# tomdbar/naqs-for-quantum-chemistry

Hardware: AMD Instinct MI355X
Metric: unique samples/sec through E_loc + log-psi eval (N2, 20 qubits) (higher is better)
Workload: dtype f32 network (f16x2-split MFMA, f32-equivalent) / f64 E_loc; 1 GPU; N2 STO-3G (20 qubits, K=2239 Pauli terms, Kxy=378), 10000 unique samples per GPU, 1xMI355X per rank; pipeline=2 independent batches in flight on 2 HIP streams (one handle pair each), batches=4 distinct key sets per rank, rotated every step, input=unique sampled bit-strings (keys) resident in HBM; random-init network, ranks=single process, no process group

## Files before the change

### include/naqs_hip.h

```cpp
#ifndef NAQS_HIP_H
#define NAQS_HIP_H

#include <stdint.h>

#ifdef __cplusplus
extern "C" {
#endif

#define NAQS_ABI_VERSION 9

typedef struct naqs_ham naqs_ham_t;

enum naqs_status {
    NAQS_OK = 0,
    NAQS_ERR_INVALID = -1,
    NAQS_ERR_HIP = -2,
    NAQS_ERR_NOMEM = -3,
    NAQS_ERR_UNSUPPORTED = -4,
    NAQS_ERR_NO_DEVICE = -5
};

enum naqs_psi_kind {
    NAQS_PSI_F32 = 0,
    NAQS_PSI_F64 = 1,
// ... 35 lines not shown

int naqs_hmatvec(naqs_ham_t *h, int64_t M, const uint64_t *keys_dev, const double *v_dev, int64_t row_begin,
                 int64_t n_rows, double *out_dev, void *stream);

int naqs_ham_connected(naqs_ham_t *h, int64_t M, const uint64_t *keys_dev, int64_t row_begin, int64_t n_rows,
                       int64_t capacity, uint64_t *out_keys_dev, int64_t *count_dev, void *stream);


int naqs_popcount_parity(const void *arr_dev, int elem_bytes, int64_t n, int8_t *out_dev, void *stream);

int naqs_get_hij(naqs_ham_t *h, int64_t M, const uint64_t *keys_dev, double *hij_dev, void *stream);

int naqs_hij_from_parity(int64_t M, int64_t Kxy, int64_t Kyz, int64_t K, const int8_t *parity_dev,
                         const int32_t *group_ptr_dev, const int32_t *term_yz_dev, const void *term_coeff_dev,
                         int coeff_bytes, void *hij_dev, void *stream);

int naqs_csr_mv(int64_t rows, const double *data_dev, const int32_t *indices_dev,
                const int32_t *indptr_dev, const double *v_dev, double *out_dev, void *stream);


int naqs_prof_enable(naqs_ham_t *h, int max_records);
int naqs_prof_read(naqs_ham_t *h, double *total_ms, int64_t *launches);
int naqs_ham_last_kernel(const naqs_ham_t *h, char *buf, int buf_len);
int naqs_prof_stride(naqs_ham_t *h, int stride);


typedef struct naqs_net naqs_net_t;

#define NAQS_NET_MAX_PAIRS 16
#define NAQS_NET_MAX_PHASE_LAYERS 8

typedef struct naqs_net_config {
    int32_t n_qubits;
    int32_t n_alpha, n_beta;
    int32_t masking;
    int32_t use_amp_spin_sym;
    int32_t amp_hidden;
    int32_t n_phase_hidden;
    int32_t phase_hidden[NAQS_NET_MAX_PHASE_LAYERS];
    int32_t qubit2model[2 * NAQS_NET_MAX_PAIRS];
    int32_t aggregate_phase;
    int32_t use_phase_spin_sym;
} naqs_net_config_t;

int naqs_net_create(const naqs_net_config_t *cfg, int device, naqs_net_t **out);
int naqs_net_create_amp_layers(const naqs_net_config_t *cfg, int32_t n_amp_hidden, int device, naqs_net_t **out);
// ... 126 lines not shown
```

### naqs-for-quantum-chemistry_amd/csrc/naqs_hip.hip

```cpp

#include <hip/hip_runtime.h>

#include <algorithm>
#include <cmath>
#include <cstdint>
#include <cstdio>
#include <cstdlib>
#include <cstring>
#include <new>
#include <numeric>
#include <type_traits>
#include <vector>

#include "naqs_common.hpp"
#include "naqs_reduce.hpp"
#include "naqs_src_hash.h"
#include "naqs_hash.hpp"
#include "naqs_poll.hpp"

#include <mutex>

namespace naqs {
thread_local hipError_t g_last_hip = hipSuccess;
thread_local char g_last_msg[200] = {0};
std::atomic<int64_t> g_launches{0};
}

namespace {

using naqs::WAVE;
using naqs::DeviceGuard;
using naqs::env_int;

constexpr int BLOCK = 256;
#ifndef NAQS_LIGHT_BATCH
#define NAQS_LIGHT_BATCH 2
#endif
constexpr int LIGHT_BATCH = NAQS_LIGHT_BATCH;
constexpr int LIGHT_BATCH_BLOOM = 4;
constexpr int queue_cap(bool bloom) { return 64 * ((bloom ? LIGHT_BATCH_BLOOM : LIGHT_BATCH) + 1); }
constexpr int LDS_BUDGET = 78 * 1024;
// ... 34 lines not shown
}

template <typename KT>
struct ElocParams {
    const KT *xy_g;
    const int32_t *row_ptr;
    const KT *yz_t;
    const double *c_t;
    int32_t Kxy, K;
    int32_t has_diag;
    int32_t light_begin;
    KT alpha_mask, beta_mask;
    int32_t n_alpha, n_beta;
    const KT *keys;
    const double2 *psi;
    const Slot<KT> *tab;
    int32_t bits;
    uint32_t tag;
    const uint32_t *bloom;
    int64_t row_begin, n_rows;
    int32_t rows_per_block;
    int32_t matvec;
    double2 *eloc;
};

using naqs::wave_sum;

__device__ __forceinline__ uint32_t to_sgpr(uint32_t v) { return (uint32_t)__builtin_amdgcn_readfirstlane((int)v); }
__device__ __forceinline__ uint64_t to_sgpr(uint64_t v) {
    const uint32_t hi = (uint32_t)__builtin_amdgcn_readfirstlane((int)(uint32_t)(v >> 32));
    const uint32_t lo = (uint32_t)__builtin_amdgcn_readfirstlane((int)(uint32_t)v);
    return ((uint64_t)hi << 32) | (uint64_t)lo;
}

__device__ __forceinline__ double2 cdiv(double2 a, double2 b) {
    double2 q;
    if (fabs(b.x) >= fabs(b.y)) {
        const double rat = b.y / b.x, scl = 1.0 / (b.x + b.y * rat);
        q.x = (a.x + a.y * rat) * scl;
        q.y = (a.y - a.x * rat) * scl;
    } else {
        const double rat = b.x / b.y, scl = 1.0 / (b.y + b.x * rat);
        q.x = (a.x * rat + a.y) * scl;
        q.y = (a.y * rat - a.x) * scl;
    }
    return q;
// ... 155 lines not shown
            while (qn >= WAVE) {
                qn -= WAVE;
                drain(qn, true);
                __builtin_amdgcn_wave_barrier();
            }
        }
        drain(0, lane < qn);
        __builtin_amdgcn_wave_barrier();

        sr = wave_sum(sr);
        si = wave_sum(si);
        if (lane == 0) {
            if (p.matvec) {
                p.eloc[r] = make_double2(sr, si);
            } else {
                const double2 q = cdiv(make_double2(sr, si), psi_i);
                p.eloc[r] = make_double2(q.x, -q.y);
            }
        }
    }

}

constexpr int PASS_BATCH = 3;
constexpr int PQ_CAP = 64 * (PASS_BATCH + 1), HQ_CAP = 128;
constexpr size_t queue_bytes_v2(int nwaves) { return (size_t)nwaves * (HQ_CAP * sizeof(int2) + PQ_CAP * sizeof(int32_t)) + 16; }

template <typename KT, int STAGE, int NT, bool BLOOM>
__global__ __launch_bounds__(NT) void eloc_kernel2(const ElocParams<KT> p) {
    constexpr int NWAVES = NT / WAVE;
    extern __shared__ __attribute__((aligned(16))) unsigned char smem[];
    double *s_c = reinterpret_cast<double *>(smem);
    int2 *s_hq = reinterpret_cast<int2 *>(s_c + (STAGE >= 2 ? p.K : 0));
    int32_t *s_pq = reinterpret_cast<int32_t *>(s_hq + NWAVES * HQ_CAP);
    int32_t *s_rp = s_pq + NWAVES * PQ_CAP + 4;
    KT *s_xy = reinterpret_cast<KT *>(s_rp + (STAGE >= 1 ? (p.Kxy + 2) & ~1 : 0));
    KT *s_yz = s_xy + (STAGE >= 1 ? p.Kxy : 0);
    uint32_t *s_bloom = reinterpret_cast<uint32_t *>(
        smem + ((reinterpret_cast<unsigned char *>(s_yz + (STAGE >= 2 ? p.K : 0)) - smem + 15) & ~15ull));

    const int tid = threadIdx.x, lane = tid & (WAVE - 1), wave = tid >> 6;

    if (BLOOM) {
        const uint4 *src = reinterpret_cast<const uint4 *>(p.bloom);
        uint4 *dst = reinterpret_cast<uint4 *>(s_bloom);
#pragma unroll 4
        for (int e = tid; e < BLOOM_WORDS / 4; e += NT) dst[e] = src[e];
    }
    if (STAGE >= 1) {
        const int n_max = STAGE >= 2 ? (p.K > p.Kxy + 1 ? p.K : p.Kxy + 1) : p.Kxy + 1;
#pragma unroll 4
        for (int t = tid; t < n_max; t += NT) {
            const bool gx = t < p.Kxy, gr = t <= p.Kxy, gt = STAGE >= 2 && t < p.K;
            const KT vx = gx ? p.xy_g[t] : (KT)0;
            const int32_t vr = gr ? p.row_ptr[t] : 0;
            KT vy = (KT)0;
            double vc = 0.0;
            if (STAGE >= 2) { vy = gt ? p.yz_t[t] : (KT)0; vc = gt ? p.c_t[t] : 0.0; }
            if (gx) s_xy[t] = vx;
            if (gr) s_rp[t] = vr;
            if (STAGE >= 2 && gt) { s_yz[t] = vy; s_c[t] = vc; }
        }
    }
    __syncthreads();

    const KT *xy = STAGE >= 1 ? s_xy : p.xy_g;
    const int32_t *rp = STAGE >= 1 ? s_rp : p.row_ptr;
    const KT *yz = STAGE >= 2 ? s_yz : p.yz_t;
    const double *cf = STAGE >= 2 ? s_c : p.c_t;
    int2 *hq = s_hq + wave * HQ_CAP;
    int32_t *pq = s_pq + wave * PQ_CAP;

    const int64_t blk_begin = (int64_t)blockIdx.x * p.rows_per_block;
    const int blk_rows = (int)min((int64_t)p.rows_per_block, p.n_rows - blk_begin);
    const bool filter = p.n_alpha >= 0;
    const Slot<KT> *__restrict__ tab = p.tab;
    const double2 *__restrict__ psi = p.psi;

    const int wave_u = __builtin_amdgcn_readfirstlane(wave);
    if (wave_u < blk_rows % NWAVES) __builtin_amdgcn_s_setprio(1);
    for (int rl = wave; rl < blk_rows; rl += NWAVES) {
        const int64_t r = blk_begin + rl;
        const int64_t i = p.row_begin + r;
        const KT key = to_sgpr(p.keys[i]);
        const double2 psi_i = psi[i];
        double sr = 0.0, si = 0.0;

        if (p.has_diag) {
            const double h = sign_sum_strided<KT>(key, yz, cf, rp[0], rp[1], lane);
            sr = h * psi_i.x;
            si = h * psi_i.y;
        }

        int qn = 0, pn = 0;
        auto drain = [&](int first, bool active) {
            if (active) {
                const int2 e = hq[first + lane];
                const double2 pj = psi[e.y];
                const int t0 = e.x & 0xFFFFFF;
                const double h = sign_sum<KT>(key, yz, cf, t0, t0 + (int)((uint32_t)e.x >> 24));
                sr += h * pj.x;
                si += h * pj.y;
            }
        };
        auto push_hits = [&](int g, int idx) {
            const unsigned long long m = __ballot(idx >= 0);
            if (m) {
                if (idx >= 0) {
                    const int pos = qn + __builtin_amdgcn_mbcnt_hi((uint32_t)(m >> 32), __builtin_amdgcn_mbcnt_lo((uint32_t)m, 0));
                    const int t0 = rp[g];
                    hq[pos] = make_int2(t0 | ((rp[g + 1] - t0) << 24), idx);
                }
                qn += __popcll(m);
                __builtin_amdgcn_wave_barrier();
                if (qn >= WAVE) {
                    qn -= WAVE;
                    drain(qn, true);
                    __builtin_amdgcn_wave_barrier();
                }
            }
        };
        auto probe_pass = [&](int first, bool active) {
            int idx = -1, g = 0;
            if (active) {
                g = pq[first + lane];
                const KT j = key ^ xy[g];
                if (!BLOOM || naqs::bloom_test<KT>(s_bloom, j)) idx = hash_find<KT>(tab, p.bits, p.tag, j);
            }
            push_hits(g, idx);
        };
        auto filter_pass = [&](int g, bool in_range) {
            bool ok = false;
            if (in_range) {
                const KT j = key ^ xy[g];
                ok = !filter || (popc((KT)(j & p.alpha_mask)) == p.n_alpha && popc((KT)(j & p.beta_mask)) == p.n_beta);
            }
            const unsigned long long m = __ballot(ok);
            if (ok) pq[pn + __builtin_amdgcn_mbcnt_hi((uint32_t)(m >> 32), __builtin_amdgcn_mbcnt_lo((uint32_t)m, 0))] = g;
            pn += __popcll(m);
        };
        int g0 = p.has_diag;
        for (; g0 + PASS_BATCH * WAVE <= p.Kxy; g0 += PASS_BATCH * WAVE) {
#pragma unroll
            for (int u = 0; u < PASS_BATCH; ++u) filter_pass(g0 + u * WAVE + lane, true);
            __builtin_amdgcn_wave_barrier();
            while (pn >= WAVE) {
                pn -= WAVE;
                probe_pass(pn, true);
            }
        }
        for (; g0 < p.Kxy; g0 += WAVE) {
            filter_pass(g0 + lane, g0 + lane < p.Kxy);
            __builtin_amdgcn_wave_barrier();
            if (pn >= WAVE) {
                pn -= WAVE;
                probe_pass(pn, true);
            }
        }
// ... 207 lines not shown
        const uint32_t n = min(*s_fill, (uint32_t)p.wg_stage);
        if (tid == 0) s_base = n ? atomicAdd(p.count, (unsigned long long)n) : 0ull;
        __syncthreads();
        const unsigned long long base = s_base;
        for (uint32_t i = tid; i < n; i += NT)
            if (base + i < cap) p.out[base + i] = (uint64_t)s_keys[i];
    }
}

}

struct naqs_ham {
    int device = 0;
    char last_kernel[96] = {0};
    int n_qubits = 0, n_alpha = -1, n_beta = -1;
    int key_bits = 32;
    int64_t K = 0, Kxy = 0;
    int32_t has_diag = 0, diag_terms = 0, n_heavy = 0;
    int32_t chunk_terms = 8;
    uint64_t alpha_mask = 0, beta_mask = 0;
    void *d_xy = nullptr, *d_yz = nullptr;
    int32_t *d_rp = nullptr, *d_col = nullptr;
    double *d_c = nullptr;
    int64_t Kxy2 = 0;
    void *d_xy2 = nullptr;
    int32_t *d_rp2 = nullptr;
    int64_t cap_M = 0;
    void *d_keys = nullptr;
    double2 *d_psi = nullptr;
    void *d_tab = nullptr;
    int64_t tab_slots = 0;
    uint32_t epoch = 0;
    uint32_t *d_bloom = nullptr;
    unsigned long long *d_seen = nullptr;
    int64_t seen_slots = 0;
    int64_t *d_conn_count = nullptr;
    int64_t *h_conn = nullptr, *d_conn_alias = nullptr;
    int64_t conn_seq = 0;
    int cu_count = 256;
    naqs::EventRing prof;
};

namespace {

int table_bits(int64_t M, size_t slot_bytes) {
    static const int64_t fmin = std::max(2, env_int("NAQS_TABLE_FACTOR", 4));
    static const int64_t fmax = std::max((int)fmin, env_int("NAQS_TABLE_MAX_FACTOR", 16));
    static const int64_t grow_bytes = (int64_t)std::max(0, env_int("NAQS_TABLE_GROW_KB", 1024)) * 1024;
    int bits = 10;
// ... 26 lines not shown
template <typename KT>
int upload_tables(naqs_ham *h, const std::vector<uint64_t> &xy_g, const std::vector<int32_t> &rp,
                  const std::vector<int32_t> &col, const std::vector<uint64_t> &yz_t,
                  const std::vector<double> &c_t) {
    std::vector<KT> xy_n(xy_g.begin(), xy_g.end()), yz_n(yz_t.begin(), yz_t.end());
    HIP_TRY(hipMalloc(&h->d_xy, std::max<size_t>(1, xy_n.size()) * sizeof(KT)));
    HIP_TRY(hipMalloc(&h->d_yz, std::max<size_t>(1, yz_n.size()) * sizeof(KT)));
    HIP_TRY(hipMalloc((void **)&h->d_rp, rp.size() * sizeof(int32_t)));
    HIP_TRY(hipMalloc((void **)&h->d_col, std::max<size_t>(1, col.size()) * sizeof(int32_t)));
    HIP_TRY(hipMemcpy(h->d_col, col.data(), col.size() * sizeof(int32_t), hipMemcpyHostToDevice));
    HIP_TRY(hipMalloc((void **)&h->d_c, std::max<size_t>(1, c_t.size()) * sizeof(double)));
    HIP_TRY(hipMemcpy(h->d_xy, xy_n.data(), xy_n.size() * sizeof(KT), hipMemcpyHostToDevice));
    HIP_TRY(hipMemcpy(h->d_yz, yz_n.data(), yz_n.size() * sizeof(KT), hipMemcpyHostToDevice));
    HIP_TRY(hipMemcpy(h->d_rp, rp.data(), rp.size() * sizeof(int32_t), hipMemcpyHostToDevice));
    HIP_TRY(hipMemcpy(h->d_c, c_t.data(), c_t.size() * sizeof(double), hipMemcpyHostToDevice));
    {
        const double oa = (double)((h->n_qubits + 1) / 2), ob = (double)(h->n_qubits / 2);
        double log2_states = (double)h->n_qubits;
        if (h->n_alpha >= 0 && h->n_beta >= 0)
            log2_states = (std::lgamma(oa + 1.0) - std::lgamma(h->n_alpha + 1.0) - std::lgamma(oa - h->n_alpha + 1.0) +
                           std::lgamma(ob + 1.0) - std::lgamma(h->n_beta + 1.0) - std::lgamma(ob - h->n_beta + 1.0)) / std::log(2.0);
        h->chunk_terms = std::min(255, std::max(1, env_int("NAQS_CHUNK_TERMS", log2_states > 20.0 ? 64 : HEAVY_TERMS)));
    }
    std::vector<KT> xy2;
    std::vector<int32_t> rp2;
    for (size_t g = 0; g + 1 < rp.size(); ++g) {
        const int32_t step = (int32_t)g < h->has_diag ? rp[g + 1] - rp[g] : h->chunk_terms;
        for (int32_t t = rp[g]; t < rp[g + 1]; t += std::max(step, 1)) { xy2.push_back(xy_n[g]); rp2.push_back(t); }
    }
    rp2.push_back(rp.back());
    h->Kxy2 = (int64_t)xy2.size();
    HIP_TRY(hipMalloc(&h->d_xy2, std::max<size_t>(1, xy2.size()) * sizeof(KT)));
    HIP_TRY(hipMalloc((void **)&h->d_rp2, rp2.size() * sizeof(int32_t)));
    HIP_TRY(hipMemcpy(h->d_xy2, xy2.data(), xy2.size() * sizeof(KT), hipMemcpyHostToDevice));
    HIP_TRY(hipMemcpy(h->d_rp2, rp2.data(), rp2.size() * sizeof(int32_t), hipMemcpyHostToDevice));
    HIP_TRY(hipDeviceSynchronize());
    return NAQS_OK;
}

int eloc_begin_impl(naqs_ham *h, int64_t M, hipStream_t s, naqs::ElocFeed *feed) {
    int st = ensure_scratch(h, M);
    if (st != NAQS_OK) return st;
    const size_t slot = h->key_bits == 32 ? sizeof(Slot<uint32_t>) : sizeof(Slot<uint64_t>);
    if (++h->epoch > 255u) {
        HIP_TRY(hipMemsetAsync(h->d_tab, 0, (size_t)h->tab_slots * slot, s));
        h->epoch = 1;
    }
    const int bloom_env = env_int("NAQS_BLOOM", -1);
    const bool use_bloom = bloom_env >= 0 ? bloom_env != 0 : (M >= 20000);
    feed->bloom = nullptr;
    if (use_bloom) {
        if (!h->d_bloom) HIP_TRY(hipMalloc((void **)&h->d_bloom, BLOOM_WORDS * sizeof(uint32_t)));
        HIP_TRY(hipMemsetAsync(h->d_bloom, 0, BLOOM_WORDS * sizeof(uint32_t), s));
        feed->bloom = h->d_bloom;
    }
    feed->tab = h->d_tab;
    feed->keys_narrow = h->d_keys;
// ... 17 lines not shown
template <typename KT>
int launch_main(naqs_ham *h, int64_t M, const naqs::ElocFeed &f, int64_t row_begin, int64_t n_rows, double *eloc_dev,
                const double *w_dev, double *out4_dev, hipStream_t s, bool matvec = false) {
    const int bits = f.bits;
    const uint32_t tag = f.tag;
    auto *tab = reinterpret_cast<Slot<KT> *>(f.tab);

    ElocParams<KT> p;
    p.xy_g = reinterpret_cast<const KT *>(h->d_xy);
    p.row_ptr = h->d_rp;
    p.yz_t = reinterpret_cast<const KT *>(h->d_yz);
    p.c_t = h->d_c;
    p.Kxy = (int32_t)h->Kxy; p.K = (int32_t)h->K;
    p.has_diag = h->has_diag;
    p.light_begin = h->has_diag + h->n_heavy;
    p.alpha_mask = (KT)h->alpha_mask; p.beta_mask = (KT)h->beta_mask;
    p.n_alpha = h->n_alpha; p.n_beta = h->n_beta;
    p.keys = reinterpret_cast<const KT *>(h->d_keys);
    p.psi = h->d_psi;
    p.tab = tab; p.bits = bits; p.tag = tag;
    p.row_begin = row_begin; p.n_rows = n_rows;
    p.eloc = reinterpret_cast<double2 *>(eloc_dev);
    p.matvec = matvec ? 1 : 0;

    const int ver = env_int("NAQS_ELOC_V", 2);
    const bool v2 = ver != 1 && h->K < (1 << 24);
    int nt = env_int("NAQS_BLOCK", 0);
    if (nt != 256 && nt != 512 && nt != 1024) nt = n_rows >= 1024 ? 1024 : 512;
    const int nwaves = nt / WAVE;
    int rpb = env_int("NAQS_ROWS_PER_BLOCK", 0);
    if (rpb <= 0) {
        const int64_t target_blocks = (int64_t)h->cu_count * (2048 / nt);
        rpb = (int)std::max<int64_t>(nwaves, (n_rows + target_blocks - 1) / target_blocks);
    }
    p.rows_per_block = rpb;

    const bool bloom = f.bloom != nullptr && nt == 1024;
    p.bloom = bloom ? f.bloom : nullptr;
    const size_t b_bytes = bloom ? (size_t)BLOOM_WORDS * sizeof(uint32_t) + 16 : 0;
    const size_t budget = bloom ? (size_t)LDS_BUDGET_BLOOM : (size_t)LDS_BUDGET;
    if (bloom) {
        const int64_t target_blocks = (int64_t)h->cu_count;
        if (env_int("NAQS_ROWS_PER_BLOCK", 0) <= 0)
            rpb = (int)std::max<int64_t>(nwaves, (n_rows + target_blocks - 1) / target_blocks);
        p.rows_per_block = rpb;
    }
    const int grid2 = (int)((n_rows + rpb - 1) / rpb);
    const int64_t Kxy_k = v2 ? h->Kxy2 : h->Kxy;
    if (v2) { p.xy_g = reinterpret_cast<const KT *>(h->d_xy2); p.row_ptr = h->d_rp2; p.Kxy = (int32_t)h->Kxy2; }
    const size_t q_bytes = v2 ? queue_bytes_v2(nwaves) : (size_t)nwaves * queue_cap(bloom) * sizeof(int2) + 16;
    const size_t g_bytes = (size_t)((Kxy_k + 2) & ~1ll) * sizeof(int32_t) + (size_t)Kxy_k * sizeof(KT);
    const size_t t_bytes = (size_t)h->K * (sizeof(double) + sizeof(KT));
    const int force = env_int("NAQS_STAGE", -1);
    int stage = (q_bytes + g_bytes + t_bytes + b_bytes <= budget) ? 2 : (q_bytes + g_bytes + b_bytes <= budget ? 1 : 0);
    if (force >= 0 && force < stage) stage = force;
    const size_t lds = q_bytes + (stage >= 1 ? g_bytes : 0) + (stage >= 2 ? t_bytes : 0) + b_bytes;

    const bool prof = h->prof.armed();
    if (prof) { int st = h->prof.begin(s); if (st != NAQS_OK) return st; }
#define NAQS_LAUNCH_K(KERNEL, ST, NTHREADS, BL)                                                                     \
    do {                                                                                                            \
        if (lds > 64 * 1024)                                               \
            (void)hipFuncSetAttribute(reinterpret_cast<const void *>(&KERNEL<KT, ST, NTHREADS, BL>),                \
                                      hipFuncAttributeMaxDynamicSharedMemorySize, (int)budget);                      \
        NAQS_KLAUNCH((KERNEL<KT, ST, NTHREADS, BL>), dim3(grid2), dim3(NTHREADS), lds, s, p);                 \
    } while (0)
#define NAQS_LAUNCH(ST, NTHREADS, BL)                                                                               \
    do {                                                                                                            \
        if (v2) NAQS_LAUNCH_K(eloc_kernel2, ST, NTHREADS, BL);                                                 \
        else NAQS_LAUNCH_K(eloc_kernel, ST, NTHREADS, BL);                                                          \
    } while (0)
#define NAQS_LAUNCH_NT(ST)                                          \
    do {                                                            \
        if (bloom) NAQS_LAUNCH(ST, 1024, true);                     \
        else if (nt == 1024) NAQS_LAUNCH(ST, 1024, false);          \
// ... 204 lines not shown
            c_d[(size_t)pos] = c_t[(size_t)t];
        }
    }
    rp_d[(size_t)Kxy] = pos;

    DeviceGuard guard;
    st = guard.init(device);
    if (st == NAQS_OK) {
        hipDeviceProp_t prop;
        if (hipGetDeviceProperties(&prop, device) == hipSuccess) h->cu_count = prop.multiProcessorCount;
        st = h->key_bits == 32 ? upload_tables<uint32_t>(h, xy_d, rp_d, col, yz_d, c_d)
                               : upload_tables<uint64_t>(h, xy_d, rp_d, col, yz_d, c_d);
    }
    if (st != NAQS_OK) { naqs_ham_destroy(h); return st; }
    *out = h;
    return NAQS_OK;
}

NAQS_API int naqs_ham_destroy(naqs_ham_t *h) {
    if (!h) return NAQS_OK;
    DeviceGuard guard;
    (void)guard.init(h->device);
    (void)h->prof.enable(0);
    void *ptrs[] = {h->d_xy, h->d_yz, h->d_rp, h->d_col, h->d_c, h->d_xy2, h->d_rp2, h->d_keys, h->d_psi, h->d_tab, h->d_bloom, h->d_seen};
    for (void *p : ptrs) if (p) (void)hipFree(p);
    if (h->d_conn_count) (void)hipFree(h->d_conn_count);
    if (h->h_conn) (void)hipHostFree(h->h_conn);
    delete h;
    return NAQS_OK;
}

NAQS_API int naqs_ham_info(const naqs_ham_t *h, int64_t info[8]) {
    if (!h || !info) return NAQS_ERR_INVALID;
    info[0] = h->K; info[1] = h->Kxy; info[2] = h->n_qubits; info[3] = h->n_alpha; info[4] = h->n_beta;
    info[5] = h->key_bits; info[6] = h->diag_terms; info[7] = h->device;
    return NAQS_OK;
}

NAQS_API int naqs_ham_reserve(naqs_ham_t *h, int64_t M) {
    if (!h || M < 0) return NAQS_ERR_INVALID;
    if (M >= (1ll << 31)) return NAQS_ERR_UNSUPPORTED;
    DeviceGuard guard;
    int st = guard.init(h->device);
    if (st != NAQS_OK) return st;
    return ensure_scratch(h, M);
}

static int eloc_common(naqs_ham_t *h, int64_t M, const uint64_t *keys_dev, const void *psi_dev, int psi_kind,
                       int64_t row_begin, int64_t n_rows, double *eloc_dev, const double *w_dev, double *out4_dev,
                       void *stream, bool matvec = false, int64_t S = 0, int64_t S_pad = 0) {
    if (!h || M < 0 || row_begin < 0 || n_rows < 0 || row_begin + n_rows > M) return NAQS_ERR_INVALID;
    if (psi_kind < NAQS_PSI_F32 || psi_kind > NAQS_LOGPSI_F64) return NAQS_ERR_INVALID;
    if (M > (int64_t)IDX_MASK) return NAQS_ERR_UNSUPPORTED;
    if ((w_dev == nullptr) != (out4_dev == nullptr)) return NAQS_ERR_INVALID;
    hipStream_t s = reinterpret_cast<hipStream_t>(stream);
    DeviceGuard guard;
    int st = guard.init(h->device);
    if (st != NAQS_OK) return st;
// ... 328 lines not shown
```

### naqs-for-quantum-chemistry_amd/naqs_amd/_lib.py

```python
import ctypes
import os

_HERE = os.path.dirname(os.path.abspath(__file__))
_LIB_DIR = os.path.join(os.path.dirname(_HERE), "lib")

NAQS_OK = 0
ABI_VERSION = 9
PSI_F32, PSI_F64, LOGPSI_F32, LOGPSI_F64 = 0, 1, 2, 3

c_i64, c_u64p, c_f64p, c_vp = ctypes.c_int64, ctypes.POINTER(ctypes.c_uint64), ctypes.POINTER(ctypes.c_double), ctypes.c_void_p

SIGNATURES = {
    "naqs_abi_version": (ctypes.c_int, []),
    "naqs_source_hash": (ctypes.c_char_p, []),
    "naqs_strerror": (ctypes.c_char_p, [ctypes.c_int]),
    "naqs_last_hip_error": (ctypes.c_int, []),
    "naqs_last_hip_error_string": (ctypes.c_char_p, []),
    "naqs_device_count": (ctypes.c_int, []),
    "naqs_device_check": (ctypes.c_int, [ctypes.c_int]),
    "naqs_net_check": (ctypes.c_int, [c_vp]),
    "naqs_terms_group": (ctypes.c_int, [c_i64, c_vp, c_vp, c_vp, ctypes.POINTER(c_i64), c_vp, c_vp, c_vp, c_vp, c_vp]),
    "naqs_ham_create": (ctypes.c_int, [ctypes.c_int, ctypes.c_int, ctypes.c_int, c_i64, c_vp, c_vp, c_vp,
                                       ctypes.c_int, ctypes.POINTER(c_vp)]),
    "naqs_ham_destroy": (ctypes.c_int, [c_vp]),
    "naqs_ham_info": (ctypes.c_int, [c_vp, ctypes.POINTER(c_i64 * 8)]),
    "naqs_ham_reserve": (ctypes.c_int, [c_vp, c_i64]),
    "naqs_eloc": (ctypes.c_int, [c_vp, c_i64, c_vp, c_vp, ctypes.c_int, c_i64, c_i64, c_vp, c_vp]),
    "naqs_eloc_reduced": (ctypes.c_int, [c_vp, c_i64, c_vp, c_vp, ctypes.c_int, c_i64, c_i64, c_vp, c_vp, c_vp, c_vp]),
    "naqs_eloc_reduce": (ctypes.c_int, [c_vp, c_i64, c_vp, c_vp, c_vp, c_vp]),
    "naqs_hmatvec": (ctypes.c_int, [c_vp, c_i64, c_vp, c_vp, c_i64, c_i64, c_vp, c_vp]),
    "naqs_ham_connected": (ctypes.c_int, [c_vp, c_i64, c_vp, c_i64, c_i64, c_i64, c_vp, c_vp, c_vp]),
    "naqs_exact_eloc": (ctypes.c_int, [c_vp, c_vp, c_i64, c_vp, c_vp, c_i64, c_i64, c_i64, c_vp, c_vp, c_vp, ctypes.POINTER(c_i64), c_vp]),
    "naqs_popcount_parity": (ctypes.c_int, [c_vp, ctypes.c_int, c_i64, c_vp, c_vp]),
    "naqs_get_hij": (ctypes.c_int, [c_vp, c_i64, c_vp, c_vp, c_vp]),
    "naqs_hij_from_parity": (ctypes.c_int, [c_i64, c_i64, c_i64, c_i64, c_vp, c_vp, c_vp, c_vp, ctypes.c_int, c_vp, c_vp]),
    "naqs_csr_mv": (ctypes.c_int, [c_i64, c_vp, c_vp, c_vp, c_vp, c_vp, c_vp]),
    "naqs_ham_last_kernel": (ctypes.c_int, [c_vp, ctypes.c_char_p, ctypes.c_int]),
    "naqs_net_last_kernel": (ctypes.c_int, [c_vp, ctypes.c_char_p, ctypes.c_int]),
    "naqs_prof_enable": (ctypes.c_int, [c_vp, ctypes.c_int]),
    "naqs_prof_read": (ctypes.c_int, [c_vp, ctypes.POINTER(ctypes.c_double), ctypes.POINTER(c_i64)]),
    "naqs_prof_stride": (ctypes.c_int, [c_vp, ctypes.c_int]),
    "naqs_net_prof_stride": (ctypes.c_int, [c_vp, ctypes.c_int]),
    "naqs_net_create": (ctypes.c_int, [c_vp, ctypes.c_int, ctypes.POINTER(c_vp)]),
    "naqs_net_create_amp_layers": (ctypes.c_int, [c_vp, ctypes.c_int32, ctypes.c_int, ctypes.POINTER(c_vp)]),
    "naqs_net_create_combined": (ctypes.c_int, [c_vp, ctypes.c_int, ctypes.POINTER(c_vp)]),
    "naqs_net_create_agg_layers": (ctypes.c_int, [c_vp, ctypes.c_int32, ctypes.c_int, ctypes.POINTER(c_vp)]),
    "naqs_net_destroy": (ctypes.c_int, [c_vp]),
    "naqs_net_param_count": (ctypes.c_int, [c_vp, ctypes.POINTER(c_i64)]),
    "naqs_net_set_weights": (ctypes.c_int, [c_vp, c_vp, c_i64, c_vp]),
    "naqs_net_logpsi": (ctypes.c_int, [c_vp, c_i64, c_vp, c_vp, c_vp]),
    "naqs_logpsi_eloc": (ctypes.c_int, [c_vp, c_vp, c_i64, c_vp, c_vp, c_vp, c_vp, c_vp, c_vp]),
    "naqs_net_prof_enable": (ctypes.c_int, [c_vp, ctypes.c_int]),
    "naqs_net_prof_read": (ctypes.c_int, [c_vp, ctypes.POINTER(ctypes.c_double), ctypes.POINTER(c_i64)]),
    "naqs_net_sample": (ctypes.c_int, [c_vp, c_i64, ctypes.c_uint64, c_i64, c_vp, c_vp, c_vp, c_vp, c_vp]),
    "naqs_net_sample_weighted": (ctypes.c_int, [c_vp, c_i64, ctypes.c_uint64, c_i64, c_vp, c_vp, c_vp, c_vp, c_vp, c_vp]),
    "naqs_net_amp_param_count": (ctypes.c_int, [c_vp, ctypes.POINTER(c_i64)]),
    "naqs_net_set_amp_weights": (ctypes.c_int, [c_vp, c_vp, c_i64, c_vp]),
    "naqs_net_logamp": (ctypes.c_int, [c_vp, c_i64, c_vp, c_vp, c_vp]),
    "naqs_net_amp_backward": (ctypes.c_int, [c_vp, c_i64, c_vp, c_vp, c_vp, c_vp]),
    "naqs_net_train_forward": (ctypes.c_int, [c_vp, c_i64, c_vp, c_vp, c_vp]),
# ... 111 lines not shown
```

### naqs-for-quantum-chemistry_amd/naqs_amd/hamiltonian.py

```python
import ctypes

import numpy as np
import torch

from . import _lib
from .packing import PackedHamiltonian, pack_qubit_hamiltonian

_KIND = {("psi", torch.float32): _lib.PSI_F32, ("psi", torch.float64): _lib.PSI_F64,
         ("log_psi", torch.float32): _lib.LOGPSI_F32, ("log_psi", torch.float64): _lib.LOGPSI_F64}


def _stream_ptr(device):
    return ctypes.c_void_p(torch.cuda.current_stream(device).cuda_stream)


def keys_to_device(keys, device):
    if isinstance(keys, np.ndarray):
        keys = torch.from_numpy(np.ascontiguousarray(keys).astype(np.uint64).view(np.int64))
    keys = keys.reshape(-1)
    if keys.dtype != torch.int64:
        keys = keys.to(torch.int64)
    return keys.to(device).contiguous()


# ... 190 lines not shown

    def dense_hij(self, keys):
        M = keys.shape[0]
        out = torch.empty((M, self.Kxy), dtype=torch.float64, device=self.device)
        st = self._lib.naqs_get_hij(self._h, M, keys.contiguous().data_ptr(), out.data_ptr(),
                                    _stream_ptr(self.device))
        _lib.check(st, "naqs_get_hij")
        return out

    def prof_enable(self, max_records, stride=1):
        _lib.check(self._lib.naqs_prof_enable(self._h, int(max_records)), "naqs_prof_enable")
        _lib.check(self._lib.naqs_prof_stride(self._h, int(stride)), "naqs_prof_stride")

    def prof_read(self):
        ms, n = ctypes.c_double(0), ctypes.c_int64(0)
        _lib.check(self._lib.naqs_prof_read(self._h, ctypes.byref(ms), ctypes.byref(n)), "naqs_prof_read")
        return ms.value, n.value

    def last_kernel(self):
        buf = ctypes.create_string_buffer(128)
        _lib.check(self._lib.naqs_ham_last_kernel(self._h, buf, 128), "naqs_ham_last_kernel")
        return buf.value.decode()


def popcount_parity_device(arr):
    if arr.dtype not in (torch.int16, torch.int32, torch.int64):
        raise TypeError(f"Unsupported array dtype for popcount_parity(...): {arr.dtype}.")
    lib = _lib.load_library()
    a = arr.contiguous()
    out = torch.empty(a.shape if a.dim() > 1 else (a.numel(), 1), dtype=torch.int8, device=a.device)
    st = lib.naqs_popcount_parity(a.data_ptr(), a.element_size(), a.numel(), out.data_ptr(), _stream_ptr(a.device))
    _lib.check(st, "naqs_popcount_parity")
    return out


def csr_mv_device(data, indices, indptr, v):
    lib = _lib.load_library()
    rows = indptr.numel() - 1
    out = torch.empty((rows, 2), dtype=torch.float64, device=v.device)
    st = lib.naqs_csr_mv(rows, data.contiguous().data_ptr(), indices.contiguous().data_ptr(),
                         indptr.contiguous().data_ptr(), v.contiguous().data_ptr(), out.data_ptr(),
                         _stream_ptr(v.device))
    _lib.check(st, "naqs_csr_mv")
    return out


# ... 49 lines not shown
```

Baseline: 352.2 million unique samples/s.

## Precompute closed-form sign tables for Pauli groups in local energy kernel

Classifies each off-diagonal Pauli group (4-flip groups whose YZ masks share a common reference, and 2-flip groups with at most one extra spectator bit) and precomputes per-group lookup tables of summed signed coefficients. At evaluation time these groups replace a per-term parity loop with one or a few table loads plus a reference parity. It also repacks the remaining terms into a compact per-chunk layout, uses a single-exit hash probe, and simplifies the electron-count filter to a total popcount. The cost is extra table memory read from global memory, added per-lane branching, and host-side classification at setup.

```diff
diff --git a/include/naqs_hip.h b/include/naqs_hip.h
--- a/include/naqs_hip.h
+++ b/include/naqs_hip.h
@@ -81,6 +81,9 @@
 int naqs_prof_enable(naqs_ham_t *h, int max_records);
 int naqs_prof_read(naqs_ham_t *h, double *total_ms, int64_t *launches);
 int naqs_ham_last_kernel(const naqs_ham_t *h, char *buf, int buf_len);
+int naqs_ham_closed_counts(const naqs_ham_t *h, int64_t out[4]);
+int naqs_closed_group(int n_qubits, uint64_t xy, int64_t n_terms, const uint64_t *yz, const double *coeff,
+                      int32_t *class_out, uint64_t *ref_out, double *table_out);
 int naqs_prof_stride(naqs_ham_t *h, int stride);
 
 
diff --git a/naqs-for-quantum-chemistry_amd/csrc/naqs_closed.hpp b/naqs-for-quantum-chemistry_amd/csrc/naqs_closed.hpp
--- /dev/null
+++ b/naqs-for-quantum-chemistry_amd/csrc/naqs_closed.hpp
@@ -0,0 +1,86 @@
+#pragma once
+#include <algorithm>
+#include <cstdint>
+#include <vector>
+
+namespace naqs {
+namespace closed {
+
+constexpr int SEG_BITS = 6;
+constexpr int SEG_SIZE = 1 << SEG_BITS;
+constexpr int MAX_UNITS = 1 << 12;
+constexpr int MAX_CLASSIFY_TERMS = 4096;
+enum { CLASS_L = 0, CLASS_D = 1, CLASS_S = 2 };
+
+struct Group {
+    int cls = CLASS_L;
+    uint64_t R = 0;
+    int pos[4] = {0, 0, 0, 0};
+};
+
+inline int popc64(uint64_t v) { return __builtin_popcountll(v); }
+inline int n_segments(int n_qubits) { return (n_qubits + SEG_BITS - 1) / SEG_BITS; }
+inline size_t d_table_doubles() { return 16; }
+inline size_t s_table_doubles(int nseg) { return (size_t)4 * (size_t)nseg * SEG_SIZE; }
+
+inline uint64_t deposit(const Group &g, int pattern, int nflip) {
+    uint64_t m = 0;
+    for (int i = 0; i < nflip; ++i)
+        if ((pattern >> i) & 1) m |= 1ull << g.pos[i];
+    return m;
+}
+
+inline Group classify(uint64_t xy, const uint64_t *yz, int n) {
+    Group g;
+    const int nflip = popc64(xy);
+    if ((nflip != 2 && nflip != 4) || n <= 0 || n > MAX_CLASSIFY_TERMS) return g;
+    int best = 1 << 30, ref = 0;
+    for (int r = 0; r < n; ++r) {
+        int worst = 0;
+        for (int t = 0; t < n; ++t) worst = std::max(worst, popc64((yz[t] ^ yz[r]) & ~xy));
+        if (worst < best) { best = worst; ref = r; }
+    }
+    if (!((nflip == 4 && best == 0) || (nflip == 2 && best <= 1))) return g;
+    g.cls = nflip == 4 ? CLASS_D : CLASS_S;
+    g.R = yz[ref];
+    for (int q = 0, k = 0; q < 64; ++q)
+        if ((xy >> q) & 1) g.pos[k++] = q;
+    return g;
+}
+
+inline uint32_t d_word(const Group &g) {
+    return (uint32_t)g.pos[0] | (uint32_t)g.pos[1] << 6 | (uint32_t)g.pos[2] << 12 | (uint32_t)g.pos[3] << 18;
+}
+inline uint32_t s_word(const Group &g, int unit) {
+    return (uint32_t)g.pos[0] | (uint32_t)g.pos[1] << 6 | (uint32_t)unit << 12;
+}
+
+inline void build_d(const Group &g, const uint64_t *yz, const double *c, int n, double *T) {
+    for (int p = 0; p < 16; ++p) {
+        const uint64_t dep = deposit(g, p, 4);
+        double acc = 0.0;
+        for (int t = 0; t < n; ++t) acc += (popc64(dep & (yz[t] ^ g.R)) & 1) ? -c[t] : c[t];
+        T[p] = acc;
+    }
+}
+
+inline void build_s(const Group &g, uint64_t xy, const uint64_t *yz, const double *c, int n, int nseg, double *B) {
+    for (int p = 0; p < 4; ++p) {
+        const uint64_t dep = deposit(g, p, 2);
+        for (int s = 0; s < nseg; ++s)
+            for (int v = 0; v < SEG_SIZE; ++v) {
+                double acc = 0.0;
+                for (int t = 0; t < n; ++t) {
+                    const uint64_t d = yz[t] ^ g.R, sp = d & ~xy;
+                    const int r = sp ? __builtin_ctzll(sp) : 0;
+                    if (r / SEG_BITS != s) continue;
+                    const int par = popc64(dep & d) + (sp ? (v >> (r - s * SEG_BITS)) & 1 : 0);
+                    acc += (par & 1) ? -c[t] : c[t];
+                }
+                B[((size_t)s * 4 + p) * SEG_SIZE + v] = acc;
+            }
+    }
+}
+
+}
+}
diff --git a/naqs-for-quantum-chemistry_amd/csrc/naqs_hip.hip b/naqs-for-quantum-chemistry_amd/csrc/naqs_hip.hip
--- a/naqs-for-quantum-chemistry_amd/csrc/naqs_hip.hip
+++ b/naqs-for-quantum-chemistry_amd/csrc/naqs_hip.hip
@@ -17,6 +17,7 @@
 #include "naqs_src_hash.h"
 #include "naqs_hash.hpp"
 #include "naqs_poll.hpp"
+#include "naqs_closed.hpp"
 
 #include <mutex>
 
@@ -97,6 +98,8 @@
     int32_t rows_per_block;
     int32_t matvec;
     double2 *eloc;
+    const double *tbl;
+    int32_t n_ref, nseg;
 };
 
 using naqs::wave_sum;
@@ -298,6 +301,25 @@
 
 }
 
+__device__ __forceinline__ uint32_t slot_val(unsigned long long kv) { return (uint32_t)kv; }
+__device__ __forceinline__ uint32_t slot_val(const naqs::Slot64Val &s) { return s.val; }
+__device__ __forceinline__ bool slot_has(unsigned long long kv, uint32_t key) { return (uint32_t)(kv >> 32) == key; }
+__device__ __forceinline__ bool slot_has(const naqs::Slot64Val &s, uint64_t key) { return s.key == key; }
+template <typename KT>
+__device__ __forceinline__ int hash_find_one_exit(const Slot<KT> *__restrict__ tab, int bits, uint32_t tag, KT key) {
+    const uint32_t mask = (1u << bits) - 1u;
+    uint32_t h = hash_key(key, bits);
+    auto s = probe_load(tab, h);
+    for (;;) {
+        const uint32_t val = slot_val(s);
+        const bool current = (val & ~IDX_MASK) == tag, hit = current && slot_has(s, key);
+        if (!current || hit) return hit ? (int)(val & IDX_MASK) : -1;
+        h = (h + 1) & mask;
+        s = probe_load(tab, h);
+    }
+}
+
+constexpr int S_BATCH = 4;
 constexpr int PASS_BATCH = 3;
 constexpr int PQ_CAP = 64 * (PASS_BATCH + 1), HQ_CAP = 128;
 constexpr size_t queue_bytes_v2(int nwaves) { return (size_t)nwaves * (HQ_CAP * sizeof(int2) + PQ_CAP * sizeof(int32_t)) + 16; }
@@ -311,7 +333,7 @@
     int32_t *s_pq = reinterpret_cast<int32_t *>(s_hq + NWAVES * HQ_CAP);
     int32_t *s_rp = s_pq + NWAVES * PQ_CAP + 4;
     KT *s_xy = reinterpret_cast<KT *>(s_rp + (STAGE >= 1 ? (p.Kxy + 2) & ~1 : 0));
-    KT *s_yz = s_xy + (STAGE >= 1 ? p.Kxy : 0);
+    KT *s_yz = s_xy + (STAGE >= 1 ? p.Kxy + p.n_ref : 0);
     uint32_t *s_bloom = reinterpret_cast<uint32_t *>(
         smem + ((reinterpret_cast<unsigned char *>(s_yz + (STAGE >= 2 ? p.K : 0)) - smem + 15) & ~15ull));
 
@@ -324,10 +346,11 @@
         for (int e = tid; e < BLOOM_WORDS / 4; e += NT) dst[e] = src[e];
     }
     if (STAGE >= 1) {
-        const int n_max = STAGE >= 2 ? (p.K > p.Kxy + 1 ? p.K : p.Kxy + 1) : p.Kxy + 1;
+        const int n_xy = p.Kxy + p.n_ref;
+        const int n_max = STAGE >= 2 ? (p.K > n_xy + 1 ? p.K : n_xy + 1) : n_xy + 1;
 #pragma unroll 4
         for (int t = tid; t < n_max; t += NT) {
-            const bool gx = t < p.Kxy, gr = t <= p.Kxy, gt = STAGE >= 2 && t < p.K;
+            const bool gx = t < n_xy, gr = t <= p.Kxy, gt = STAGE >= 2 && t < p.K;
             const KT vx = gx ? p.xy_g[t] : (KT)0;
             const int32_t vr = gr ? p.row_ptr[t] : 0;
             KT vy = (KT)0;
@@ -344,12 +367,14 @@
     const int32_t *rp = STAGE >= 1 ? s_rp : p.row_ptr;
     const KT *yz = STAGE >= 2 ? s_yz : p.yz_t;
     const double *cf = STAGE >= 2 ? s_c : p.c_t;
+    const double *__restrict__ tbl = p.tbl;
     int2 *hq = s_hq + wave * HQ_CAP;
     int32_t *pq = s_pq + wave * PQ_CAP;
 
     const int64_t blk_begin = (int64_t)blockIdx.x * p.rows_per_block;
     const int blk_rows = (int)min((int64_t)p.rows_per_block, p.n_rows - blk_begin);
     const bool filter = p.n_alpha >= 0;
+    const int n_total = p.n_alpha + p.n_beta;
     const Slot<KT> *__restrict__ tab = p.tab;
     const double2 *__restrict__ psi = p.psi;
 
@@ -363,7 +388,7 @@
         double sr = 0.0, si = 0.0;
 
         if (p.has_diag) {
-            const double h = sign_sum_strided<KT>(key, yz, cf, rp[0], rp[1], lane);
+            const double h = sign_sum_strided<KT>(key, yz, cf, 0, rp[0], lane);
             sr = h * psi_i.x;
             si = h * psi_i.y;
         }
@@ -373,8 +398,35 @@
             if (active) {
                 const int2 e = hq[first + lane];
                 const double2 pj = psi[e.y];
-                const int t0 = e.x & 0xFFFFFF;
-                const double h = sign_sum<KT>(key, yz, cf, t0, t0 + (int)((uint32_t)e.x >> 24));
+                double h;
+                if ((uint32_t)e.x >> 24) {
+                    const int t0 = e.x & 0xFFFFFF;
+                    h = sign_sum<KT>(key, yz, cf, t0, t0 + (int)((uint32_t)e.x >> 24));
+                } else {
+                    const uint32_t w = (uint32_t)rp[e.x];
+                    const int par = popc((KT)(key & xy[p.Kxy + e.x]));
+                    const uint32_t b0 = (uint32_t)(key >> (w & 63u)) & 1u, b1 = (uint32_t)(key >> ((w >> 6) & 63u)) & 1u;
+                    const uint32_t b2 = (uint32_t)(key >> ((w >> 12) & 63u)) & 1u, b3 = (uint32_t)(key >> ((w >> 18) & 63u)) & 1u;
+                    const bool cls_s = popc(xy[e.x]) == 2;
+                    const uint32_t s_off = ((((w >> 12) & 0xFFFu) + (b0 | b1 << 1)) << naqs::closed::SEG_BITS);
+                    const double *__restrict__ tp = tbl + (cls_s ? s_off : (uint32_t)e.x * 16u);
+                    h = tp[cls_s ? ((uint32_t)key & (uint32_t)(naqs::closed::SEG_SIZE - 1)) : (b0 | b1 << 1 | b2 << 2 | b3 << 3)];
+                    if (cls_s) {
+                        for (int sg0 = 1; sg0 < p.nseg; sg0 += S_BATCH) {
+                            double part[S_BATCH];
+#pragma unroll
+                            for (int u = 0; u < S_BATCH; ++u) {
+                                const int sg = sg0 + u;
+                                part[u] = sg < p.nseg ? tp[(uint32_t)(sg << (naqs::closed::SEG_BITS + 2)) +
+                                                           ((uint32_t)(key >> (sg * naqs::closed::SEG_BITS)) & (uint32_t)(naqs::closed::SEG_SIZE - 1))]
+                                                      : 0.0;
+                            }
+#pragma unroll
+                            for (int u = 0; u < S_BATCH; ++u) h += part[u];
+                        }
+                    }
+                    h = signed_term(h, par);
+                }
                 sr += h * pj.x;
                 si += h * pj.y;
             }
@@ -384,8 +436,8 @@
             if (m) {
                 if (idx >= 0) {
                     const int pos = qn + __builtin_amdgcn_mbcnt_hi((uint32_t)(m >> 32), __builtin_amdgcn_mbcnt_lo((uint32_t)m, 0));
-                    const int t0 = rp[g];
-                    hq[pos] = make_int2(t0 | ((rp[g + 1] - t0) << 24), idx);
+                    const uint32_t w = (uint32_t)rp[g];
+                    hq[pos] = make_int2(w < 0x01000000u ? g : (int)w, idx);
                 }
                 qn += __popcll(m);
                 __builtin_amdgcn_wave_barrier();
@@ -401,7 +453,7 @@
             if (active) {
                 g = pq[first + lane];
                 const KT j = key ^ xy[g];
-                if (!BLOOM || naqs::bloom_test<KT>(s_bloom, j)) idx = hash_find<KT>(tab, p.bits, p.tag, j);
+                if (!BLOOM || naqs::bloom_test<KT>(s_bloom, j)) idx = hash_find_one_exit<KT>(tab, p.bits, p.tag, j);
             }
             push_hits(g, idx);
         };
@@ -409,7 +461,7 @@
             bool ok = false;
             if (in_range) {
                 const KT j = key ^ xy[g];
-                ok = !filter || (popc((KT)(j & p.alpha_mask)) == p.n_alpha && popc((KT)(j & p.beta_mask)) == p.n_beta);
+                ok = !filter || (popc((KT)(j & p.alpha_mask)) == p.n_alpha && popc(j) == n_total);
             }
             const unsigned long long m = __ballot(ok);
             if (ok) pq[pn + __builtin_amdgcn_mbcnt_hi((uint32_t)(m >> 32), __builtin_amdgcn_mbcnt_lo((uint32_t)m, 0))] = g;
@@ -663,9 +715,13 @@
     void *d_xy = nullptr, *d_yz = nullptr;
     int32_t *d_rp = nullptr, *d_col = nullptr;
     double *d_c = nullptr;
-    int64_t Kxy2 = 0;
-    void *d_xy2 = nullptr;
+    int64_t Kxy2 = 0, K2 = 0;
+    void *d_xy2 = nullptr, *d_yz2 = nullptr;
     int32_t *d_rp2 = nullptr;
+    double *d_c2 = nullptr, *d_tbl = nullptr;
+    int32_t closed_on = 1;
+    int32_t nseg = 1, n_ref = 0;
+    int64_t n_class_d = 0, n_class_s = 0, n_class_l = 0, tbl_bytes = 0;
     int64_t cap_M = 0;
     void *d_keys = nullptr;
     double2 *d_psi = nullptr;
@@ -738,17 +794,82 @@
                            std::lgamma(ob + 1.0) - std::lgamma(h->n_beta + 1.0) - std::lgamma(ob - h->n_beta + 1.0)) / std::log(2.0);
         h->chunk_terms = std::min(255, std::max(1, env_int("NAQS_CHUNK_TERMS", log2_states > 20.0 ? 64 : HEAVY_TERMS)));
     }
-    std::vector<KT> xy2;
+    namespace cf = naqs::closed;
+    const size_t n_groups = rp.size() - 1;
+    h->closed_on = env_int("NAQS_ELOC_CLOSED", 1) != 0 ? 1 : 0;
+    h->nseg = cf::n_segments(h->n_qubits);
+    const size_t max_bytes = (size_t)std::max(0, env_int("NAQS_CLOSED_MAX_KB", 4096)) * 1024;
+    std::vector<cf::Group> cls(n_groups);
+    size_t bytes = 0, n_closed = 0;
+    for (size_t g = (size_t)h->has_diag; g < n_groups; ++g) {
+        const int n = rp[g + 1] - rp[g];
+        cf::Group c;
+        if (h->closed_on) c = cf::classify(xy_g[g], yz_t.data() + rp[g], n);
+        if (c.cls == cf::CLASS_D && n > h->chunk_terms) c.cls = cf::CLASS_L;
+        const size_t add = (cf::d_table_doubles() + (c.cls == cf::CLASS_S ? cf::s_table_doubles(h->nseg) : 0)) * sizeof(double);
+        if (c.cls != cf::CLASS_L && bytes + add > max_bytes) c.cls = cf::CLASS_L;
+        if (c.cls != cf::CLASS_L) { bytes += add; ++n_closed; }
+        cls[g] = c;
+    }
+    const size_t d_units = (((size_t)h->has_diag + n_closed) * cf::d_table_doubles() + cf::SEG_SIZE - 1) / cf::SEG_SIZE;
+    const size_t s_units = cf::s_table_doubles(h->nseg) / cf::SEG_SIZE;
+    size_t units = d_units;
+    std::vector<int32_t> unit_of(n_groups, 0);
+    h->n_class_d = h->n_class_s = h->n_class_l = 0;
+    for (size_t g = (size_t)h->has_diag; g < n_groups; ++g) {
+        cf::Group &c = cls[g];
+        if (c.cls == cf::CLASS_S) {
+            if (units + s_units > (size_t)cf::MAX_UNITS) c.cls = cf::CLASS_L;
+            else { unit_of[g] = (int32_t)units; units += s_units; }
+        }
+        (c.cls == cf::CLASS_D ? h->n_class_d : c.cls == cf::CLASS_S ? h->n_class_s : h->n_class_l) += 1;
+    }
+    std::vector<KT> xy2, ref2, yz2;
     std::vector<int32_t> rp2;
-    for (size_t g = 0; g + 1 < rp.size(); ++g) {
-        const int32_t step = (int32_t)g < h->has_diag ? rp[g + 1] - rp[g] : h->chunk_terms;
-        for (int32_t t = rp[g]; t < rp[g + 1]; t += std::max(step, 1)) { xy2.push_back(xy_n[g]); rp2.push_back(t); }
-    }
-    rp2.push_back(rp.back());
+    std::vector<double> c2;
+    std::vector<double> tbl(h->n_class_d + h->n_class_s > 0 ? units * cf::SEG_SIZE : 0, 0.0);
+    if (h->has_diag) {
+        xy2.push_back(xy_n[0]); ref2.push_back((KT)0); rp2.push_back(rp[1] - rp[0]);
+        for (int32_t t = rp[0]; t < rp[1]; ++t) { yz2.push_back(yz_n[t]); c2.push_back(c_t[t]); }
+    }
+    for (size_t g = (size_t)h->has_diag; g < n_groups; ++g) {
+        const cf::Group &c = cls[g];
+        if (c.cls == cf::CLASS_L) continue;
+        const int n = rp[g + 1] - rp[g];
+        const size_t v = xy2.size();
+        xy2.push_back(xy_n[g]); ref2.push_back((KT)c.R);
+        if (c.cls == cf::CLASS_D) {
+            rp2.push_back((int32_t)cf::d_word(c));
+            cf::build_d(c, yz_t.data() + rp[g], c_t.data() + rp[g], n, tbl.data() + v * cf::d_table_doubles());
+        } else {
+            rp2.push_back((int32_t)cf::s_word(c, unit_of[g]));
+            cf::build_s(c, xy_g[g], yz_t.data() + rp[g], c_t.data() + rp[g], n, h->nseg, tbl.data() + (size_t)unit_of[g] * cf::SEG_SIZE);
+        }
+    }
+    for (size_t g = (size_t)h->has_diag; g < n_groups; ++g) {
+        if (cls[g].cls != cf::CLASS_L) continue;
+        for (int32_t t = rp[g]; t < rp[g + 1]; t += h->chunk_terms) {
+            const int32_t n = std::min(h->chunk_terms, rp[g + 1] - t);
+            xy2.push_back(xy_n[g]);
+            rp2.push_back((int32_t)((uint32_t)yz2.size() | (uint32_t)n << 24));
+            for (int32_t u = t; u < t + n; ++u) { yz2.push_back(yz_n[u]); c2.push_back(c_t[u]); }
+        }
+    }
+    rp2.push_back(0);
     h->Kxy2 = (int64_t)xy2.size();
+    h->n_ref = h->n_class_d + h->n_class_s > 0 ? (int32_t)ref2.size() : 0;
+    xy2.insert(xy2.end(), ref2.begin(), ref2.begin() + h->n_ref);
+    h->K2 = (int64_t)yz2.size();
+    h->tbl_bytes = (int64_t)(tbl.size() * sizeof(double));
     HIP_TRY(hipMalloc(&h->d_xy2, std::max<size_t>(1, xy2.size()) * sizeof(KT)));
+    HIP_TRY(hipMalloc(&h->d_yz2, std::max<size_t>(1, yz2.size()) * sizeof(KT)));
+    HIP_TRY(hipMalloc((void **)&h->d_c2, std::max<size_t>(1, c2.size()) * sizeof(double)));
+    HIP_TRY(hipMalloc((void **)&h->d_tbl, std::max<size_t>(1, tbl.size()) * sizeof(double)));
     HIP_TRY(hipMalloc((void **)&h->d_rp2, rp2.size() * sizeof(int32_t)));
     HIP_TRY(hipMemcpy(h->d_xy2, xy2.data(), xy2.size() * sizeof(KT), hipMemcpyHostToDevice));
+    HIP_TRY(hipMemcpy(h->d_yz2, yz2.data(), yz2.size() * sizeof(KT), hipMemcpyHostToDevice));
+    HIP_TRY(hipMemcpy(h->d_c2, c2.data(), c2.size() * sizeof(double), hipMemcpyHostToDevice));
+    HIP_TRY(hipMemcpy(h->d_tbl, tbl.data(), tbl.size() * sizeof(double), hipMemcpyHostToDevice));
     HIP_TRY(hipMemcpy(h->d_rp2, rp2.data(), rp2.size() * sizeof(int32_t), hipMemcpyHostToDevice));
     HIP_TRY(hipDeviceSynchronize());
     return NAQS_OK;
@@ -812,6 +933,7 @@
     p.row_begin = row_begin; p.n_rows = n_rows;
     p.eloc = reinterpret_cast<double2 *>(eloc_dev);
     p.matvec = matvec ? 1 : 0;
+    p.tbl = h->d_tbl; p.nseg = h->nseg; p.n_ref = 0;
 
     const int ver = env_int("NAQS_ELOC_V", 2);
     const bool v2 = ver != 1 && h->K < (1 << 24);
@@ -837,10 +959,13 @@
     }
     const int grid2 = (int)((n_rows + rpb - 1) / rpb);
     const int64_t Kxy_k = v2 ? h->Kxy2 : h->Kxy;
-    if (v2) { p.xy_g = reinterpret_cast<const KT *>(h->d_xy2); p.row_ptr = h->d_rp2; p.Kxy = (int32_t)h->Kxy2; }
+    if (v2) {
+        p.xy_g = reinterpret_cast<const KT *>(h->d_xy2); p.row_ptr = h->d_rp2; p.Kxy = (int32_t)h->Kxy2;
+        p.yz_t = reinterpret_cast<const KT *>(h->d_yz2); p.c_t = h->d_c2; p.K = (int32_t)h->K2; p.n_ref = h->n_ref;
+    }
     const size_t q_bytes = v2 ? queue_bytes_v2(nwaves) : (size_t)nwaves * queue_cap(bloom) * sizeof(int2) + 16;
-    const size_t g_bytes = (size_t)((Kxy_k + 2) & ~1ll) * sizeof(int32_t) + (size_t)Kxy_k * sizeof(KT);
-    const size_t t_bytes = (size_t)h->K * (sizeof(double) + sizeof(KT));
+    const size_t g_bytes = (size_t)((Kxy_k + 2) & ~1ll) * sizeof(int32_t) + (size_t)(Kxy_k + (v2 ? h->n_ref : 0)) * sizeof(KT);
+    const size_t t_bytes = (size_t)(v2 ? h->K2 : h->K) * (sizeof(double) + sizeof(KT));
     const int force = env_int("NAQS_STAGE", -1);
     int stage = (q_bytes + g_bytes + t_bytes + b_bytes <= budget) ? 2 : (q_bytes + g_bytes + b_bytes <= budget ? 1 : 0);
     if (force >= 0 && force < stage) stage = force;
@@ -1091,7 +1216,7 @@
     DeviceGuard guard;
     (void)guard.init(h->device);
     (void)h->prof.enable(0);
-    void *ptrs[] = {h->d_xy, h->d_yz, h->d_rp, h->d_col, h->d_c, h->d_xy2, h->d_rp2, h->d_keys, h->d_psi, h->d_tab, h->d_bloom, h->d_seen};
+    void *ptrs[] = {h->d_xy, h->d_yz, h->d_rp, h->d_col, h->d_c, h->d_xy2, h->d_rp2, h->d_yz2, h->d_c2, h->d_tbl, h->d_keys, h->d_psi, h->d_tab, h->d_bloom, h->d_seen};
     for (void *p : ptrs) if (p) (void)hipFree(p);
     if (h->d_conn_count) (void)hipFree(h->d_conn_count);
     if (h->h_conn) (void)hipHostFree(h->h_conn);
@@ -1103,6 +1228,24 @@
     if (!h || !info) return NAQS_ERR_INVALID;
     info[0] = h->K; info[1] = h->Kxy; info[2] = h->n_qubits; info[3] = h->n_alpha; info[4] = h->n_beta;
     info[5] = h->key_bits; info[6] = h->diag_terms; info[7] = h->device;
+    return NAQS_OK;
+}
+
+NAQS_API int naqs_closed_group(int n_qubits, uint64_t xy, int64_t n_terms, const uint64_t *yz, const double *coeff,
+                               int32_t *class_out, uint64_t *ref_out, double *table_out) {
+    if (n_qubits <= 0 || n_qubits > 64 || n_terms <= 0 || n_terms >= (1ll << 31) || !yz || !coeff || !class_out || !ref_out) return NAQS_ERR_INVALID;
+    namespace cf = naqs::closed;
+    const cf::Group g = cf::classify(xy, yz, (int)n_terms);
+    *class_out = g.cls;
+    *ref_out = g.R;
+    if (table_out && g.cls == cf::CLASS_D) cf::build_d(g, yz, coeff, (int)n_terms, table_out);
+    if (table_out && g.cls == cf::CLASS_S) cf::build_s(g, xy, yz, coeff, (int)n_terms, cf::n_segments(n_qubits), table_out);
+    return NAQS_OK;
+}
+
+NAQS_API int naqs_ham_closed_counts(const naqs_ham_t *h, int64_t out[4]) {
+    if (!h || !out) return NAQS_ERR_INVALID;
+    out[0] = h->n_class_d; out[1] = h->n_class_s; out[2] = h->n_class_l; out[3] = h->tbl_bytes;
     return NAQS_OK;
 }
 
diff --git a/naqs-for-quantum-chemistry_amd/naqs_amd/_lib.py b/naqs-for-quantum-chemistry_amd/naqs_amd/_lib.py
--- a/naqs-for-quantum-chemistry_amd/naqs_amd/_lib.py
+++ b/naqs-for-quantum-chemistry_amd/naqs_amd/_lib.py
@@ -36,6 +36,9 @@
     "naqs_hij_from_parity": (ctypes.c_int, [c_i64, c_i64, c_i64, c_i64, c_vp, c_vp, c_vp, c_vp, ctypes.c_int, c_vp, c_vp]),
     "naqs_csr_mv": (ctypes.c_int, [c_i64, c_vp, c_vp, c_vp, c_vp, c_vp, c_vp]),
     "naqs_ham_last_kernel": (ctypes.c_int, [c_vp, ctypes.c_char_p, ctypes.c_int]),
+    "naqs_closed_group": (ctypes.c_int, [ctypes.c_int, ctypes.c_uint64, c_i64, c_vp, c_vp, ctypes.POINTER(ctypes.c_int32),
+                                         ctypes.POINTER(ctypes.c_uint64), c_vp]),
+    "naqs_ham_closed_counts": (ctypes.c_int, [c_vp, ctypes.POINTER(c_i64 * 4)]),
     "naqs_net_last_kernel": (ctypes.c_int, [c_vp, ctypes.c_char_p, ctypes.c_int]),
     "naqs_prof_enable": (ctypes.c_int, [c_vp, ctypes.c_int]),
     "naqs_prof_read": (ctypes.c_int, [c_vp, ctypes.POINTER(ctypes.c_double), ctypes.POINTER(c_i64)]),
diff --git a/naqs-for-quantum-chemistry_amd/naqs_amd/hamiltonian.py b/naqs-for-quantum-chemistry_amd/naqs_amd/hamiltonian.py
--- a/naqs-for-quantum-chemistry_amd/naqs_amd/hamiltonian.py
+++ b/naqs-for-quantum-chemistry_amd/naqs_amd/hamiltonian.py
@@ -236,6 +236,11 @@
         _lib.check(self._lib.naqs_ham_last_kernel(self._h, buf, 128), "naqs_ham_last_kernel")
         return buf.value.decode()
 
+    def closed_counts(self):
+        out = (ctypes.c_int64 * 4)()
+        _lib.check(self._lib.naqs_ham_closed_counts(self._h, ctypes.byref(out)), "naqs_ham_closed_counts")
+        return tuple(int(v) for v in out)
+
 
 def popcount_parity_device(arr):
     if arr.dtype not in (torch.int16, torch.int32, torch.int64):
```

Measured after the change: 360.0 million unique samples/s, median of 6. 2.2% higher.
